# zailaiyiwan123/NOVA_pointcloud

Hardware: AMD Instinct MI355X
Metric: generated points/sec/node, NOVA-d48w1024 @2048 pts, 64-step sample (higher is better)
Workload: dtype bf16; 1 GPU; d48w1024_2048pts_b32; ar_steps=64, diffusion_steps=25, batch_per_gpu=32, global_batch=32, guidance=cfg 2-pass, process_group=none

## Files before the change

### include/nova_hip.h

```cpp
#ifndef NOVA_HIP_H_
#define NOVA_HIP_H_

#ifdef __cplusplus
extern "C" {
#endif

#define NOVA_HIP_VERSION 403

typedef enum { NOVA_F32 = 0, NOVA_BF16 = 1, NOVA_F16 = 2 } nova_dtype;
typedef enum { NOVA_ACT_NONE = 0, NOVA_ACT_GELU_ERF = 1, NOVA_ACT_SILU = 2 } nova_act;
typedef enum {
  NOVA_OK = 0,
  NOVA_ERR_ARG = -1,
  NOVA_ERR_SHAPE = -2,
  NOVA_ERR_LAUNCH = -3,
  NOVA_ERR_DEVICE = -4
} nova_status;

int nova_version(void);
const char* nova_last_error(void);
int nova_check_device(void);

#define NOVA_PROF_SLOTS 10
int nova_prof_enable(int on);
int nova_prof_collect(double* ms, double* work, long long* launches, int slots);

int nova_debug_force_gemm_tile(int tile);

int nova_debug_set_attn_variant(int variant);

int nova_debug_set_graphs(int on);
int nova_debug_graph_stats(long* captures, long* replays);
int nova_debug_drop_graphs(void);

int nova_gemm_bias_act(const void* A, const void* W, const float* bias, void* out, int M, int N, int K, int act,
                       int dtype, void* stream);

int nova_quantize_rows_fp8(const void* x_bf16, void* out_fp8, float* scale, long long rows, int D, void* stream);
int nova_gemm_fp8_bias_act(const void* A8, const float* a_scale, const void* W8, const float* w_scale, const float* bias,
                           void* out_bf16, int M, int N, int K, int act, void* stream);

int nova_qkv_rope(const void* x, const void* Wqkv, const float* bias, const float* rope, void* qkv, int S, int L, int D,
                  int heads, int rope_batch, int dtype, void* stream);

int nova_qkv_rope_cols(const void* x, const void* W, const float* bias, const float* rope, void* out, int M, int N, int K,
                       int L, int rope_batch, int head_dim, int rope_cols, int dtype, void* stream);

int nova_rope_table(const float* pos, const long long* ids, float* rope, int nb, int pad, int n_tok, int n_pos, int hd,
                    const float* inv_freq, void* stream);

int nova_attn_fwd(const void* q, const void* k, const void* v, void* o, int S, int heads, int Lq, int Lk, int head_dim,
                  long q_row_stride, long kv_row_stride, long o_row_stride, float scale, int dtype, void* stream);

int nova_attn_fwd_lse(const void* q_scaled, const void* k, const void* v, void* o, float* lse, int S, int heads, int L,
                      int head_dim, long qkv_row_stride, long o_row_stride, const int* key_limit, void* stream);
int nova_attn_bwd(const void* q_scaled, const void* k, const void* v, const void* o, const void* d_o, const float* lse,
                  float* delta_scratch, void* dq, void* dk, void* dv, int S, int heads, int L, int head_dim,
                  long qkv_row_stride, long o_row_stride, long do_row_stride, long dqkv_row_stride, float scale,
                  const int* key_limit, void* stream);

int nova_act_fwd(const void* x, void* y, long long n, int kind, int dtype, void* stream);
int nova_act_bwd(const void* x, const void* dy, void* dx, long long n, int kind, int dtype, void* stream);

int nova_row_norm_bwd(const void* x, const void* dy, const float* gamma, const float* beta, const void* mod, long mod_ld,
                      int scale_off, int shift_off, int gate_off, void* dx, void* dmod, float* dgamma_part, float* dbeta_part,
                      int parts, long rows, int D, float eps, int dtype, void* stream);

int nova_row_norm(const void* in, void* out, const float* gamma, const float* beta, const void* mod, long mod_ld,
                  int scale_off, int shift_off, int gate_off, const void* res, const int* gather, long rows, int D,
                  float eps, int dtype, void* stream);

int nova_row_norm_chain(const void* g, const void* x, const float* gamma, const float* beta, const void* mod, long mod_ld,
                        int gate_off, int scale_off, int shift_off, float eps_first, float eps_second, void* x_new_out,
                        void* h_out, long rows, int D, int dtype, void* stream);

int nova_adaln_fc1(const void* x, const void* mod, long mod_ld, int scale_off, int shift_off, float eps, const void* w,
                   const float* bias, void* h, void* out, long rows, int N, int D, int act, int dtype, void* stream);

int nova_embed_canvas(const float* canvas, const float* mask, const void* w, const float* bias, const void* mask_token,
                      const void* pos_embed, void* z0, int B, int N, int P, int D, int dtype, void* stream);
// ... 105 lines not shown
```

### nova_pointcloud_amd/csrc/capi.hip

```cpp
#include <cstdarg>
#include <cstdio>
#include <cstring>
#include <atomic>
#include <cmath>
#include <cstdlib>
#include <mutex>
#include <string>
#include <unordered_map>
#include <utility>
#include <vector>
#include "common.h"
#include "nova_internal.h"

namespace nova {

static thread_local char g_err[512] = "";

int set_error(int code, const char* fmt, ...) {
  va_list ap;
  va_start(ap, fmt);
  vsnprintf(g_err, sizeof(g_err), fmt, ap);
  va_end(ap);
  return code;
}

int check_launch(const char* what) {
  const hipError_t e = hipGetLastError();
  if (e == hipSuccess) return 0;
  return set_error(NOVA_ERR_LAUNCH, "%s: %s", what, hipGetErrorString(e));
}

struct ProfRec { hipEvent_t a, b; int slot; double work; };
static std::atomic<bool> g_prof_on{false};
static std::mutex g_prof_mu;
static std::vector<ProfRec> g_prof;
static std::vector<std::pair<hipEvent_t, hipEvent_t>> g_prof_pool;

ProfScope::ProfScope(int slot, double work, hipStream_t s) : idx(-1), st(s) {
  if (!g_prof_on.load(std::memory_order_relaxed)) return;
  std::lock_guard<std::mutex> lk(g_prof_mu);
  ProfRec r;
  if (!g_prof_pool.empty()) {
    r.a = g_prof_pool.back().first;
    r.b = g_prof_pool.back().second;
    g_prof_pool.pop_back();
  } else if (hipEventCreate(&r.a) != hipSuccess || hipEventCreate(&r.b) != hipSuccess) {
    return;
  }
  r.slot = slot;
  r.work = work;
  (void)hipEventRecord(r.a, st);
  g_prof.push_back(r);
  idx = (int)g_prof.size() - 1;
}
ProfScope::~ProfScope() {
  if (idx < 0) return;
  std::lock_guard<std::mutex> lk(g_prof_mu);
  if (idx < (int)g_prof.size()) (void)hipEventRecord(g_prof[idx].b, st);
}

static inline bool bad_dtype(int dtype) { return dtype != NOVA_F32 && dtype != NOVA_BF16 && dtype != NOVA_F16; }
static inline size_t esize(int dtype) { return dtype_is16(dtype) ? 2 : 4; }

}

using namespace nova;

#define NOVA_REQUIRE(cond, code, ...) \
  do {                                \
    if (!(cond)) return set_error(code, __VA_ARGS__); \
  } while (0)
#define NOVA_TRY(expr)        \
  do {                        \
    const int rc_ = (expr);   \
    if (rc_ != 0) return rc_; \
  } while (0)

namespace nova {
static thread_local bool g_walk_rev = false;
void walk_reverse(bool on) { g_walk_rev = on; }
bool walk_is_reverse() { return g_walk_rev; }
#ifdef NOVA_EXPERIMENTS
static int g_walk_alternate = 1;
void walk_set_alternate(int on) { g_walk_alternate = on; }
#else
constexpr int g_walk_alternate = 1;
#endif
}

extern "C" {

int nova_version(void) { return NOVA_HIP_VERSION; }
const char* nova_last_error(void) { return g_err; }

int nova_check_device(void) {
  int dev = -1;
  if (hipGetDevice(&dev) != hipSuccess) return set_error(NOVA_ERR_DEVICE, "no HIP device");
  hipDeviceProp_t prop;
  if (hipGetDeviceProperties(&prop, dev) != hipSuccess) return set_error(NOVA_ERR_DEVICE, "hipGetDeviceProperties failed");
  if (strncmp(prop.gcnArchName, "gfx950", 6) != 0)
    return set_error(NOVA_ERR_DEVICE, "device %d is %s; libnova_hip is built for gfx950 only", dev, prop.gcnArchName);
  return 0;
}

int nova_debug_force_gemm_tile(int tile) {
  NOVA_REQUIRE(gemm_force_tile(tile) == 0, NOVA_ERR_ARG,
               "force_gemm_tile: this build knows 0 (auto), 16 (small-M kernel; 161 / 162 / 164 with 16 / 32 / 64 rows per workgroup), 64 / 128 (the small-M tile kernels), 256 (persistent), 257 (one tile per workgroup) and 258 (persistent, prologue form); experiment codes need the NOVA_EXPERIMENTS build");
  return 0;
}

int nova_prof_enable(int on) {
  g_prof_on.store(on != 0);
  return 0;
}

int nova_prof_collect(double* ms, double* work, long long* launches, int slots) {
  NOVA_REQUIRE(ms && work && launches && slots >= PROF_SLOTS, NOVA_ERR_ARG, "prof_collect: need %d slots", PROF_SLOTS);
  for (int i = 0; i < slots; ++i) { ms[i] = 0; work[i] = 0; launches[i] = 0; }
  std::lock_guard<std::mutex> lk(g_prof_mu);
  for (auto& r : g_prof) {
    float t = 0.f;
    if (hipEventSynchronize(r.b) == hipSuccess && hipEventElapsedTime(&t, r.a, r.b) == hipSuccess) {
      ms[r.slot] += t;
      work[r.slot] += r.work;
      launches[r.slot] += 1;
    }
    g_prof_pool.emplace_back(r.a, r.b);
  }
  g_prof.clear();
  return 0;
}

int nova_gemm_bias_act(const void* A, const void* W, const float* bias, void* out, int M, int N, int K, int act,
                       int dtype, void* stream) {
  NOVA_REQUIRE(!bad_dtype(dtype), NOVA_ERR_ARG, "gemm: bad dtype %d", dtype);
  NOVA_REQUIRE(M == 0 || (A && W && out), NOVA_ERR_ARG, "gemm: null pointer");
  return gemm_bias_act(A, W, bias, out, M, N, K, act, dtype, (hipStream_t)stream);
}

int nova_quantize_rows_fp8(const void* x, void* out, float* scale, long long rows, int D, void* stream) {
  NOVA_REQUIRE(rows <= 0 || (x && out && scale), NOVA_ERR_ARG, "quantize_rows_fp8: null pointer");
  return quantize_rows_fp8(x, out, scale, (long)rows, D, (hipStream_t)stream);
}

int nova_gemm_fp8_bias_act(const void* A8, const float* a_scale, const void* W8, const float* w_scale, const float* bias,
                           void* out, int M, int N, int K, int act, void* stream) {
  NOVA_REQUIRE(M <= 0 || (A8 && a_scale && W8 && w_scale && out), NOVA_ERR_ARG, "gemm_fp8: null pointer");
  NOVA_REQUIRE(act >= NOVA_ACT_NONE && act <= NOVA_ACT_SILU, NOVA_ERR_ARG, "gemm_fp8: bad activation %d", act);
  return gemm256_fp8_launch(A8, a_scale, W8, w_scale, bias, out, M, N, K, act, (hipStream_t)stream);
}

int nova_qkv_rope(const void* x, const void* Wqkv, const float* bias, const float* rope, void* qkv, int S, int L, int D,
                  int heads, int rope_batch, int dtype, void* stream) {
  NOVA_REQUIRE(!bad_dtype(dtype), NOVA_ERR_ARG, "qkv_rope: bad dtype %d", dtype);
  NOVA_REQUIRE(S * L == 0 || (x && Wqkv && qkv), NOVA_ERR_ARG, "qkv_rope: null pointer");
  return gemm_qkv_rope(x, Wqkv, bias, rope, qkv, S, L, D, heads, rope_batch, dtype, (hipStream_t)stream);
}

int nova_qkv_rope_cols(const void* x, const void* W, const float* bias, const float* rope, void* out, int M, int N, int K,
                       int L, int rope_batch, int head_dim, int rope_cols, int dtype, void* stream) {
// ... 530 lines not shown
```

### nova_pointcloud_amd/csrc/gemm.hip

```cpp
#include <cstdlib>
#include "common.h"
#include "nova_internal.h"

namespace nova {

constexpr int ROWB = 128;

struct GemmEpi {
  const float* bias;
  const float* rope;
  int L;
  int rope_batch;
  int hd;
  int rope_cols;
  float q_scale;
  int q_cols;
};

enum { EPI_NONE = 0, EPI_GELU = 1, EPI_SILU = 2, EPI_ROPE = 3 };

template <typename T> struct Frag;
template <> struct Frag<bf16_t> { u4v v; };
template <> struct Frag<f16_t> { u4v v; };
template <> struct Frag<float> { f4v v; };

__device__ __forceinline__ f4v mma(const Frag<bf16_t>& w, const Frag<bf16_t>& a, f4v c) { return Half16<bf16_t>::mfma16(w.v, a.v, c); }
__device__ __forceinline__ f4v mma(const Frag<f16_t>& w, const Frag<f16_t>& a, f4v c) { return Half16<f16_t>::mfma16(w.v, a.v, c); }
__device__ __forceinline__ f4v mma(const Frag<float>& w, const Frag<float>& a, f4v c) {
#pragma unroll
  for (int j = 0; j < 4; ++j) c = __builtin_amdgcn_mfma_f32_16x16x4f32(w.v[j], a.v[j], c, 0, 0, 0);
  return c;
}

template <typename T>
__device__ __forceinline__ Frag<T> lds_frag(const char* tile, int row, int chunk) {
  const int phys = chunk ^ ((row >> 1) & 7);
  Frag<T> f;
  f.v = *reinterpret_cast<const decltype(f.v)*>(tile + row * ROWB + phys * 16);
  return f;
}

#ifndef NOVA_GEMM64_STAGES
#define NOVA_GEMM64_STAGES 2
#endif
template <typename T, int EPI, int F = 4>
__global__ __launch_bounds__(256, 2) void gemm_kernel(const T* __restrict__ A, const T* __restrict__ W,
                                                       T* __restrict__ C, int M, int N, int K, int ntm,
                                                       int ntn, GemmEpi e) {
  constexpr int BM = 32 * F, BN = 32 * F, TILE_BYTES = BM * ROWB, WT = 16 * F;
  constexpr int NST = F == 2 ? NOVA_GEMM64_STAGES : 2;
  __shared__ __attribute__((aligned(16))) char smem[NST * 2 * TILE_BYTES];
  const int tid = threadIdx.x, lane = tid & 63, wid = tid >> 6;
  const int wm = wid >> 1, wn = wid & 1;

  const int nwg = ntm * ntn;
  const int t = xcd_remap(blockIdx.x, nwg);
  constexpr int GM = 8;
  const int per_group = GM * ntn;
  const int group = t / per_group, first_m = group * GM;
  const int gsz = min(ntm - first_m, GM);
  const int tm = first_m + (t % per_group) % gsz;
  const int tn = (t % per_group) / gsz;
  const int m0 = tm * BM, n0 = tn * BN;

  const int rr = lane >> 3, cp = lane & 7;
  const char* a_src[4];
  const char* w_src[4];
  const size_t rowbytes = (size_t)K * sizeof(T);
#pragma unroll
// ... 20 lines not shown
  f4v bv[F];
#pragma unroll
  for (int nf = 0; nf < F; ++nf) bv[nf] = f4v{0.f, 0.f, 0.f, 0.f};
  if (e.bias) {
#pragma unroll
    for (int nf = 0; nf < F; ++nf) bv[nf] = *reinterpret_cast<const f4v*>(e.bias + n0 + wn * WT + nf * 16 + fg * 4);
  }
  f4v acc[F][F];
#pragma unroll
  for (int i = 0; i < F; ++i)
#pragma unroll
    for (int j = 0; j < F; ++j) acc[i][j] = bv[i];

#pragma unroll
  for (int s = 0; s < NST - 1; ++s)
    if (s < nkt) stage(s, s);
  for (int kt = 0; kt < nkt; ++kt) {
    if constexpr (NST == 2) {
      asm volatile("s_waitcnt vmcnt(0)" ::: "memory");
    } else {
      const int young = min(NST - 2, nkt - 1 - kt);
      if (young >= 3) asm volatile("s_waitcnt vmcnt(%0)" ::"n"(3 * 2 * F) : "memory");
      else if (young == 2) asm volatile("s_waitcnt vmcnt(%0)" ::"n"(2 * 2 * F) : "memory");
      else if (young == 1) asm volatile("s_waitcnt vmcnt(%0)" ::"n"(1 * 2 * F) : "memory");
      else asm volatile("s_waitcnt vmcnt(0)" ::: "memory");
    }
    if constexpr (NST == 2) __syncthreads();
    else asm volatile("s_barrier" ::: "memory");
    if (kt + NST - 1 < nkt) stage((kt + NST - 1) % NST, kt + NST - 1);
    const char* ta = smem + (kt % NST) * 2 * TILE_BYTES;
    const char* tw = ta + TILE_BYTES;
#pragma unroll
    for (int kk = 0; kk < 2; ++kk) {
      Frag<T> af[F], wf[F];
#pragma unroll
      for (int f = 0; f < F; ++f) {
        af[f] = lds_frag<T>(ta, wm * WT + f * 16 + fr, fg + 4 * kk);
        wf[f] = lds_frag<T>(tw, wn * WT + f * 16 + fr, fg + 4 * kk);
      }
#pragma unroll
      for (int nf = 0; nf < F; ++nf)
#pragma unroll
        for (int mf = 0; mf < F; ++mf) acc[nf][mf] = mma(wf[nf], af[mf], acc[nf][mf]);
    }
  }

  const bool rot = EPI == EPI_ROPE && n0 < e.rope_cols;
#pragma unroll
  for (int mf = 0; mf < F; ++mf) {
    const int m = m0 + wm * WT + mf * 16 + fr;
    if (m >= M) continue;
    f4v cs[F];
    if (rot) {
      const int s = m / e.L, l = m - s * e.L;
      const float* ropem = e.rope + ((size_t)(s % e.rope_batch) * e.L + l) * e.hd;
#pragma unroll
      for (int nf = 0; nf < F; ++nf) cs[nf] = *reinterpret_cast<const f4v*>(ropem + (n0 + wn * WT + nf * 16 + fg * 4) % e.hd);
    }
    T* dst = C + (size_t)m * N + n0 + wn * WT + fg * 4;
#pragma unroll
    for (int nf = 0; nf < F; ++nf) {
      f4v v = acc[nf][mf];
      if (EPI == EPI_GELU) {
#pragma unroll
        for (int j = 0; j < 4; ++j) v[j] = sizeof(T) == 2 ? v[j] : gelu_erf(v[j]);
        if (sizeof(T) == 2) v = gelu_erf_fast4(v);
      } else if (EPI == EPI_SILU) {
#pragma unroll
        for (int j = 0; j < 4; ++j) v[j] = silu(v[j]);
      } else if (EPI == EPI_ROPE) {
        if (rot) {
          v = rope_rotate4(v, cs[nf]);
        }
        if (n0 < e.q_cols) v = v * e.q_scale;
      }
      if constexpr (sizeof(T) == 2) {
        u2v o = {Half16<T>::pack(v[0], v[1]), Half16<T>::pack(v[2], v[3])};
        *reinterpret_cast<u2v*>(dst + nf * 16) = o;
      } else {
        *reinterpret_cast<f4v*>(dst + nf * 16) = v;
      }
    }
  }
}

int gemm256_launch(const void* A, const void* W, void* C, int M, int N, int K, int epi, const float* bias,
                   const float* rope, int L, int rope_batch, int hd, int rope_cols, float q_scale, int q_cols, int dtype,
                   hipStream_t st, int form = 0);
int gemm256_cu_count();

static thread_local int g_force_tile = 0;
#ifdef NOVA_EXPERIMENTS
void gemm256_set_variant(int v);
void gemm256_set_gm(int g);
void gemm256_set_stagger(int cycles);
void gemm256_set_grid(int n);
void walk_set_alternate(int on);
#endif
int gemm_forced_tile() { return g_force_tile; }
int gemm_force_tile(int tile) {
#ifdef NOVA_EXPERIMENTS
  if (tile == 50000 || tile == 50001) {
    walk_set_alternate(tile - 50000);
    return 0;
  }
  if (tile >= 40000 && tile <= 40512) {
    gemm256_set_grid(tile - 40000);
    return 0;
  }
  if (tile >= 30000 && tile < 31000) {
    gemm256_set_stagger((tile - 30000) * 256);
    return 0;
  }
  if (tile >= 7001 && tile <= 7064) {
    gemm256_set_gm(tile - 7000);
    return 0;
  }
  if (tile >= 2560 && tile <= 2580) {
    gemm256_set_variant(tile - 2560);
    tile = 256;
  }
#endif
  if (tile == 161 || tile == 162 || tile == 164) {
    skinny_force_row_blocks(tile - 160);
    tile = 16;
  } else {
    skinny_force_row_blocks(0);
  }
  if (tile != 0 && tile != 16 && tile != 64 && tile != 128 && tile != 256 && tile != 257 && tile != 258) return -1;
  g_force_tile = tile;
  return 0;
}

static long min_tiles256() {
  static const long v = [] {
    const char* e = getenv("NOVA_GEMM_MIN_TILES");
    return e && *e ? atol(e) : (long)gemm256_cu_count() / 2;
  }();
  return v;
}

template <typename T>
static int launch_gemm(const void* A, const void* W, void* C, int M, int N, int K, int epi, const GemmEpi& e,
                       hipStream_t st) {
  const int kelems = ROWB / (int)sizeof(T);
  if (M <= 0) return 0;
  if (N % 128 != 0 || K % kelems != 0 || K <= 0)
    return set_error(NOVA_ERR_SHAPE, "gemm: need N %% 128 == 0 and K %% %d == 0 (got M=%d N=%d K=%d)", kelems, M, N, K);
  const bool can256 = N % 256 == 0 && (epi != EPI_ROPE || (e.rope_cols % 256 == 0 && e.q_cols % 256 == 0));
  if (g_force_tile >= 256 && !can256) return set_error(NOVA_ERR_SHAPE, "gemm: 256-tile kernel needs N %% 256 == 0");
  const long tiles256 = (long)((M + 255) / 256) * (N / 256);
  if (can256 && (g_force_tile >= 256 || (g_force_tile == 0 && M >= 4096 && tiles256 >= min_tiles256())))
    return gemm256_launch(A, W, C, M, N, K, epi, e.bias, e.rope, e.L, e.rope_batch, e.hd, e.rope_cols, e.q_scale, e.q_cols,
                          dtype_of<T>(), st, g_force_tile == 257 ? 1 : g_force_tile == 258 ? 2 : 0);
  constexpr int BM = 128, BN = 128;
  int ntm = (M + BM - 1) / BM, ntn = N / BN;
  ProfScope prof(PROF_GEMM_SMALL, 2.0 * M * N * K, st);
  const T* a = static_cast<const T*>(A);
  const T* w = static_cast<const T*>(W);
  T* c = static_cast<T*>(C);
  static const bool tile64_ok = [] { const char* v = getenv("NOVA_GEMM_TILE64"); return !(v && v[0] == '0'); }();
  if (g_force_tile == 64 || (tile64_ok && g_force_tile == 0 && epi != EPI_ROPE && (long)ntm * ntn * 4 <= (long)gemm256_cu_count() * 3)) {
    if (epi == EPI_ROPE) return set_error(NOVA_ERR_SHAPE, "gemm: the 64 tile has no RoPE epilogue");
    ntm = (M + 63) / 64;
    ntn = N / 64;
    dim3 grid64(ntm * ntn), block(256);
    switch (epi) {
      case EPI_NONE: hipLaunchKernelGGL((gemm_kernel<T, EPI_NONE, 2>), grid64, block, 0, st, a, w, c, M, N, K, ntm, ntn, e); break;
      case EPI_GELU: hipLaunchKernelGGL((gemm_kernel<T, EPI_GELU, 2>), grid64, block, 0, st, a, w, c, M, N, K, ntm, ntn, e); break;
      case EPI_SILU: hipLaunchKernelGGL((gemm_kernel<T, EPI_SILU, 2>), grid64, block, 0, st, a, w, c, M, N, K, ntm, ntn, e); break;
      default: return set_error(NOVA_ERR_ARG, "gemm: unknown epilogue %d", epi);
    }
    return check_launch("gemm (64 tile)");
  }
  dim3 grid(ntm * ntn), block(256);
  switch (epi) {
    case EPI_NONE: hipLaunchKernelGGL((gemm_kernel<T, EPI_NONE>), grid, block, 0, st, a, w, c, M, N, K, ntm, ntn, e); break;
    case EPI_GELU: hipLaunchKernelGGL((gemm_kernel<T, EPI_GELU>), grid, block, 0, st, a, w, c, M, N, K, ntm, ntn, e); break;
    case EPI_SILU: hipLaunchKernelGGL((gemm_kernel<T, EPI_SILU>), grid, block, 0, st, a, w, c, M, N, K, ntm, ntn, e); break;
    case EPI_ROPE: hipLaunchKernelGGL((gemm_kernel<T, EPI_ROPE>), grid, block, 0, st, a, w, c, M, N, K, ntm, ntn, e); break;
    default: return set_error(NOVA_ERR_ARG, "gemm: unknown epilogue %d", epi);
  }
  return check_launch("gemm");
}

int gemm_bias_act(const void* A, const void* W, const float* bias, void* out, int M, int N, int K, int act,
                  int dtype, hipStream_t st) {
  GemmEpi e{bias, nullptr, 1, 1, 2, 0, 1.0f, 0};
  if (act < 0 || act > 2) return set_error(NOVA_ERR_ARG, "gemm: unknown activation %d", act);
  if (dtype_is16(dtype) && (g_force_tile == 16 || (g_force_tile == 0 && skinny_gemm_fits(M, N, K, false))))
    return skinny_gemm(A, W, bias, out, M, N, K, act, nullptr, dtype, st);
  return dispatch_dtype(dtype, [&](auto tag) { return launch_gemm<decltype(tag)>(A, W, out, M, N, K, act, e, st); });
}

bool gemm_modulate_fused(int M, int N, int K, int dtype) {
  return dtype_is16(dtype) && (g_force_tile == 16 || (g_force_tile == 0 && skinny_gemm_fits(M, N, K, true)));
}

int gemm_modulate_act(const RowNormArgs& pro, const void* W, const float* bias, void* out, int M, int N, int K, int act,
                      int dtype, hipStream_t st) {
  if (gemm_modulate_fused(M, N, K, dtype)) return skinny_gemm(nullptr, W, bias, out, M, N, K, act, &pro, dtype, st);
  if (int rc = row_norm(pro, dtype, st)) return rc;
  return gemm_bias_act(pro.out, W, bias, out, M, N, K, act, dtype, st);
}

int gemm_qkv_rope(const void* x, const void* Wqkv, const float* bias, const float* rope, void* qkv, int S, int L,
                  int D, int heads, int rope_batch, int dtype, hipStream_t st, float q_scale) {
  const int hd = D / heads;
  if (heads <= 0 || D % heads != 0 || hd % 4 != 0) return set_error(NOVA_ERR_SHAPE, "qkv_rope: bad heads/D");
  const int epi = (rope || q_scale != 1.0f) ? EPI_ROPE : EPI_NONE;
  if (rope && rope_batch <= 0) return set_error(NOVA_ERR_ARG, "qkv_rope: rope_batch must be > 0");
  GemmEpi e{bias, rope, L, rope ? rope_batch : 1, hd, rope ? 2 * D : 0, q_scale, q_scale != 1.0f ? D : 0};
  return dispatch_dtype(dtype, [&](auto tag) { return launch_gemm<decltype(tag)>(x, Wqkv, qkv, S * L, 3 * D, D, epi, e, st); });
}

int gemm_rope_cols(const void* x, const void* W, const float* bias, const float* rope, void* out, int M, int N, int K,
                   int L, int rope_batch, int hd, int rope_cols, int dtype, hipStream_t st) {
  if (rope && rope_batch <= 0) return set_error(NOVA_ERR_ARG, "rope_cols: rope_batch must be > 0");
  GemmEpi e{bias, rope, L, rope ? rope_batch : 1, hd, rope_cols, 1.0f, 0};
  const int epi = rope ? EPI_ROPE : EPI_NONE;
  return dispatch_dtype(dtype, [&](auto tag) { return launch_gemm<decltype(tag)>(x, W, out, M, N, K, epi, e, st); });
}

}
```

### nova_pointcloud_amd/csrc/gemm256.hip

```cpp
#include <type_traits>
#ifndef NOVA_GEMM_ACT_ROWS
#define NOVA_GEMM_ACT_ROWS 1
#endif
#include "common.h"
#include "nova_internal.h"

namespace nova {

constexpr int P_UNIT = 128 * 128;
constexpr int P_BUF = 4 * P_UNIT;
constexpr int P_KLDS = 2 * P_BUF;
constexpr int P_BIAS = P_KLDS;
constexpr int P_LDS = P_KLDS + 1024;

struct GemmEpi;
struct GemmEpi256 {
  const float* bias;
  const float* rope;
  int L, rope_batch, hd, rope_cols;
  float q_scale;
  int q_cols;
  int gm;
  int rev;
  const float* sa;
// ... 932 lines not shown
#ifdef NOVA_EXPERIMENTS
static int g_gm256 = 8;
static int g_stagger256 = 0;
void gemm256_set_stagger(int cycles) { g_stagger256 = cycles; }
void gemm256_set_gm(int g) { g_gm256 = g; }
static int g_var256 = 20;
void gemm256_set_variant(int v) { g_var256 = v; }
#else
constexpr int g_gm256 = 8;
constexpr int g_stagger256 = 0;
constexpr int g_var256 = 20;
#endif

template <typename T, int VAR>
static int launch256v(const void* A, const void* W, void* C, int M, int N, int K, int epi, const GemmEpi256& e,
                     hipStream_t st) {
  const int ntm = (M + 255) / 256, ntn = N / 256;
  dim3 grid(ntm * ntn), block(512);
  ProfScope prof(prof_gemm_slot(epi, N, K), 2.0 * M * N * K, st);
  const T* a = static_cast<const T*>(A);
  const T* w = static_cast<const T*>(W);
  T* c = static_cast<T*>(C);
  switch (epi) {
    case E_NONE: hipLaunchKernelGGL((gemm256_kernel<T, E_NONE, VAR>), grid, block, 0, st, a, w, c, M, N, K, ntm, ntn, e); break;
    case E_GELU: hipLaunchKernelGGL((gemm256_kernel<T, E_GELU, VAR>), grid, block, 0, st, a, w, c, M, N, K, ntm, ntn, e); break;
    case E_SILU: hipLaunchKernelGGL((gemm256_kernel<T, E_SILU, VAR>), grid, block, 0, st, a, w, c, M, N, K, ntm, ntn, e); break;
    case E_ROPE: hipLaunchKernelGGL((gemm256_kernel<T, E_ROPE, VAR>), grid, block, 0, st, a, w, c, M, N, K, ntm, ntn, e); break;
    default: return set_error(NOVA_ERR_ARG, "gemm256: unknown epilogue %d", epi);
  }
  return check_launch("gemm256");
}

#ifdef NOVA_EXPERIMENTS
static int g_grid256 = 0;
void gemm256_set_grid(int n) { g_grid256 = n & ~7; }
#else
constexpr int g_grid256 = 0;
#endif
static int cu_slots() {
  if (g_grid256 > 0) return g_grid256;
  static int n = 0;
  if (n == 0) {
    int dev = 0, cus = 0;
    if (hipGetDevice(&dev) != hipSuccess || hipDeviceGetAttribute(&cus, hipDeviceAttributeMultiprocessorCount, dev) != hipSuccess || cus < 8) cus = 256;
    n = cus & ~7;
  }
  return n;
}

int gemm256_cu_count() { return cu_slots(); }

template <typename T>
static int launch256p(const void* A, const void* W, void* C, int M, int N, int K, int epi, const GemmEpi256& e,
                      hipStream_t st) {
  const int ntm = (M + 255) / 256, ntn = N / 256;
  dim3 grid(cu_slots()), block(512);
  ProfScope prof(prof_gemm_slot(epi, N, K), 2.0 * M * N * K, st);
  const T* a = static_cast<const T*>(A);
  const T* w = static_cast<const T*>(W);
  T* c = static_cast<T*>(C);
  switch (epi) {
    case E_NONE: hipLaunchKernelGGL((gemm256p_kernel<T, E_NONE>), grid, block, 0, st, a, w, c, M, N, K, ntm, ntn, e); break;
    case E_GELU: hipLaunchKernelGGL((gemm256p_kernel<T, E_GELU>), grid, block, 0, st, a, w, c, M, N, K, ntm, ntn, e); break;
    case E_SILU: hipLaunchKernelGGL((gemm256p_kernel<T, E_SILU>), grid, block, 0, st, a, w, c, M, N, K, ntm, ntn, e); break;
    case E_ROPE: hipLaunchKernelGGL((gemm256p_kernel<T, E_ROPE>), grid, block, 0, st, a, w, c, M, N, K, ntm, ntn, e); break;
    default: return set_error(NOVA_ERR_ARG, "gemm256: unknown epilogue %d", epi);
  }
  return check_launch("gemm256p");
}

int gemm256_fp8_launch(const void* A8, const float* sa, const void* W8, const float* sw, const float* bias, void* C, int M,
                       int N, int K, int epi, hipStream_t st, const float* rope, int L, int rope_batch, int hd, int rope_cols,
                       float q_scale, int q_cols, int sa_scalar, const float* q8_scale, unsigned* q8_amax) {
  if (M <= 0) return 0;
  if (N % 256 != 0 || K % 128 != 0 || K <= 0) return set_error(NOVA_ERR_SHAPE, "gemm_fp8: need N %% 256 == 0 and K %% 128 == 0 (got N=%d K=%d)", N, K);
  if (epi == E_ROPE && (rope_cols % 256 || q_cols % 256 || (rope && (L < 16 || rope_batch <= 0 || hd <= 0))))
    return set_error(NOVA_ERR_SHAPE, "gemm_fp8: RoPE epilogue needs rope_cols, q_cols %% 256 == 0 and L >= 16");
  GemmEpi256 e{bias, rope, rope ? L : 1, rope ? rope_batch : 1, rope ? hd : 2, rope ? rope_cols : 0, q_scale, q_cols, g_gm256,
               walk_is_reverse() ? 1 : 0, sa, sw, 0};
  e.sa_scalar = sa_scalar;
  e.q8_scale = q8_scale;
  e.q8_amax = q8_amax;
  if (epi == E_GELU_Q8 && (!q8_scale || !q8_amax)) return set_error(NOVA_ERR_ARG, "gemm_fp8: the e4m3-output epilogue needs a scale and an amax word");
  const int ntm = (M + 255) / 256, ntn = N / 256;
  dim3 grid(cu_slots()), block(512);
  ProfScope prof(prof_gemm_slot(epi == E_GELU_Q8 ? E_GELU : epi, N, K), 2.0 * M * N * K, st);
  const fp8_t* a = static_cast<const fp8_t*>(A8);
  const fp8_t* w = static_cast<const fp8_t*>(W8);
  bf16_t* c = static_cast<bf16_t*>(C);
  switch (epi) {
    case E_NONE: hipLaunchKernelGGL((gemm256p_kernel<fp8_t, E_NONE>), grid, block, 0, st, a, w, c, M, N, K, ntm, ntn, e); break;
    case E_GELU: hipLaunchKernelGGL((gemm256p_kernel<fp8_t, E_GELU>), grid, block, 0, st, a, w, c, M, N, K, ntm, ntn, e); break;
    case E_SILU: hipLaunchKernelGGL((gemm256p_kernel<fp8_t, E_SILU>), grid, block, 0, st, a, w, c, M, N, K, ntm, ntn, e); break;
    case E_ROPE: hipLaunchKernelGGL((gemm256p_kernel<fp8_t, E_ROPE>), grid, block, 0, st, a, w, c, M, N, K, ntm, ntn, e); break;
    case E_GELU_Q8: hipLaunchKernelGGL((gemm256p_kernel<fp8_t, E_GELU_Q8>), grid, block, 0, st, a, w, c, M, N, K, ntm, ntn, e); break;
    default: return set_error(NOVA_ERR_ARG, "gemm_fp8: unknown epilogue %d", epi);
  }
  return check_launch("gemm256p fp8");
}

template <typename T>
static int launch256c(const void* A, const void* W, void* C, int M, int N, int K, int epi, const GemmEpi256& e,
                      hipStream_t st) {
  const int ntm = (M + 255) / 256, ntn = N / 256;
  dim3 grid(cu_slots()), block(512);
  ProfScope prof(prof_gemm_slot(epi, N, K), 2.0 * M * N * K, st);
  const T* a = static_cast<const T*>(A);
  const T* w = static_cast<const T*>(W);
  T* c = static_cast<T*>(C);
  switch (epi) {
    case E_NONE: hipLaunchKernelGGL((gemm256c_kernel<T, E_NONE>), grid, block, 0, st, a, w, c, M, N, K, ntm, ntn, e); break;
    case E_GELU: hipLaunchKernelGGL((gemm256c_kernel<T, E_GELU>), grid, block, 0, st, a, w, c, M, N, K, ntm, ntn, e); break;
    case E_SILU: hipLaunchKernelGGL((gemm256c_kernel<T, E_SILU>), grid, block, 0, st, a, w, c, M, N, K, ntm, ntn, e); break;
    case E_ROPE:
      if (e.rope && e.hd == 64) hipLaunchKernelGGL((gemm256c_kernel<T, E_ROPE, true>), grid, block, 0, st, a, w, c, M, N, K, ntm, ntn, e);
      else hipLaunchKernelGGL((gemm256c_kernel<T, E_ROPE, false>), grid, block, 0, st, a, w, c, M, N, K, ntm, ntn, e);
      break;
    default: return set_error(NOVA_ERR_ARG, "gemm256: unknown epilogue %d", epi);
  }
  return check_launch("gemm256c");
}

template <typename T>
static int launch256(const void* A, const void* W, void* C, int M, int N, int K, int epi, const GemmEpi256& e,
                     hipStream_t st, int form) {
  if (form != 1 && g_var256 == 20 && !(epi == E_ROPE && e.rope && e.L < 16)) {
    const int nkt = K / (128 / (int)sizeof(T));
    if (form == 0 && nkt >= 4 && (nkt & 1) == 0) return launch256c<T>(A, W, C, M, N, K, epi, e, st);
    return launch256p<T>(A, W, C, M, N, K, epi, e, st);
  }
#ifdef NOVA_EXPERIMENTS
  switch (g_var256) {
    case 1: return launch256v<T, 1>(A, W, C, M, N, K, epi, e, st);
    case 3: return launch256v<T, 3>(A, W, C, M, N, K, epi, e, st);
    case 0: return launch256v<T, 0>(A, W, C, M, N, K, epi, e, st);
    case 10: return launch256v<T, 10>(A, W, C, M, N, K, epi, e, st);
    case 11: return launch256v<T, 11>(A, W, C, M, N, K, epi, e, st);
    case 12: return launch256v<T, 12>(A, W, C, M, N, K, epi, e, st);
    default: break;
  }
#endif
  return launch256v<T, 2>(A, W, C, M, N, K, epi, e, st);
}

int gemm256_launch(const void* A, const void* W, void* C, int M, int N, int K, int epi, const float* bias,
                   const float* rope, int L, int rope_batch, int hd, int rope_cols, float q_scale, int q_cols, int dtype,
                   hipStream_t st, int form) {
#ifdef NOVA_EXPERIMENTS
  const int gm = g_gm256;
#else
  const int gm = (N <= 1024 && K * (int)(dtype_is16(dtype) ? 2 : 4) <= 2048) ? 16 : g_gm256;
#endif
  GemmEpi256 e{bias, rope, L, rope_batch, hd, rope_cols, q_scale, q_cols, gm, walk_is_reverse() ? 1 : 0, nullptr, nullptr, g_stagger256};
  return dispatch_dtype(dtype, [&](auto tag) { return launch256<decltype(tag)>(A, W, C, M, N, K, epi, e, st, form); });
}

}
```

### nova_pointcloud_amd/csrc/nova_internal.h

```cpp
#pragma once
#include <hip/hip_runtime.h>
#include "../../include/nova_hip.h"

#include "common.h"

namespace nova {

template <typename T> constexpr int dtype_of() { return sizeof(T) == 4 ? NOVA_F32 : NOVA_BF16; }
template <> constexpr int dtype_of<f16_t>() { return NOVA_F16; }
inline bool dtype_is16(int dtype) { return dtype == NOVA_BF16 || dtype == NOVA_F16; }
template <typename F> inline auto dispatch_dtype(int dtype, F&& f) {
  return dtype == NOVA_BF16 ? f(bf16_t{}) : dtype == NOVA_F16 ? f(f16_t{}) : f(float{});
}
template <typename F> inline auto dispatch_half(int dtype, F&& f) { return dtype == NOVA_F16 ? f(f16_t{}) : f(bf16_t{}); }

int set_error(int code, const char* fmt, ...) __attribute__((format(printf, 2, 3)));
int check_launch(const char* what);

enum { PROF_GEMM_NONE = 0, PROF_GEMM_GELU, PROF_GEMM_SILU, PROF_GEMM_ROPE, PROF_ATTN, PROF_ROWNORM, PROF_GEMM_SMALL, PROF_GEMM_WIDEK,
       PROF_TOKENS, PROF_DECODER, PROF_SLOTS };
inline int prof_gemm_slot(int epi, int N, int K) { return epi == 0 && K > N ? PROF_GEMM_WIDEK : PROF_GEMM_NONE + epi; }
struct ProfScope {
  ProfScope(int slot, double work, hipStream_t st);
  ~ProfScope();
  int idx;
  hipStream_t st;
};

int gemm_bias_act(const void* A, const void* W, const float* bias, void* out, int M, int N, int K, int act,
                  int dtype, hipStream_t st);
int gemm_qkv_rope(const void* x, const void* Wqkv, const float* bias, const float* rope, void* qkv, int S, int L,
                  int D, int heads, int rope_batch, int dtype, hipStream_t st, float q_scale = 1.0f);

int gemm_rope_cols(const void* x, const void* W, const float* bias, const float* rope, void* out, int M, int N, int K,
                   int L, int rope_batch, int hd, int rope_cols, int dtype, hipStream_t st);
int gemm_force_tile(int tile);
int gemm_forced_tile();
void walk_reverse(bool on);
bool walk_is_reverse();

int attn_fwd(const void* q, const void* k, const void* v, void* o, int S, int heads, int Lq, int Lk, int hd,
             long q_row_stride, long kv_row_stride, long o_row_stride, float scale, int dtype, hipStream_t st,
             bool q_prescaled = false, long kv_seq_stride = 0, float* lse = nullptr, const int* klim = nullptr);
int attn_fwd_m16(const void* q, const void* k, const void* v, void* o, int S, int heads, int Lq, int Lk, int hd, long q_rs, long kv_rs,
                 long o_rs, float cl, int dtype, hipStream_t st, long kv_ss, float* lse, int rows_per_wave, bool sum_on_mfma, bool pipelined = false,
                 const int* klim = nullptr);
constexpr int NOVA_ATTN_DEFAULT_VARIANT = 3;
int attn_set_variant(int v);
int attn_variant();
int attn_bwd(const void* q, const void* k, const void* v, const void* o, const void* d_o, const float* lse, float* delta, void* dq,
             void* dk, void* dv, int S, int heads, int L, int hd, long qkv_rs, long o_rs, long do_rs, long dqkv_rs, float scale,
             hipStream_t st, const int* klim = nullptr);

struct RowNormArgs {
  const void* in;
  void* out;
  const float* gamma;
  const float* beta;
  const void* mod;
  long mod_ld;
  int scale_off, shift_off, gate_off;
  const void* res;
  const int* gather;
  long rows;
  int D;
  float eps;
  int rev = 0;
  void* out8 = nullptr;
  float* out8_scale = nullptr;
};
int row_norm(const RowNormArgs& a, int dtype, hipStream_t st);

bool skinny_gemm_fits(int M, int N, int K, bool modulate);
bool gemm_modulate_fused(int M, int N, int K, int dtype);
int skinny_forced_row_blocks();
void skinny_force_row_blocks(int rb);
int skinny_gemm(const void* A, const void* W, const float* bias, void* out, int M, int N, int K, int act,
                const RowNormArgs* pro, int dtype, hipStream_t st);
int row_norm_chain(const RowNormArgs& a2, const RowNormArgs& a1, void* x_new_out, int dtype, hipStream_t st);
int gemm_modulate_act(const RowNormArgs& pro, const void* W, const float* bias, void* out, int M, int N, int K, int act,
                      int dtype, hipStream_t st);

int rope_table(const float* pos, const long long* ids, float* table, int nb, int pad, int n_tok, int n_pos,
               int hd, const float* inv_freq, hipStream_t st);
int embed_canvas(const float* canvas, const float* mask, const void* w, const float* bias, const void* mask_token,
                 const void* pos_embed, void* z0, int B, int N, int P, int D, int dtype, hipStream_t st);
int build_sequence(const void* prefix, long prefix_seq_rows, const void* tokens, long tok_batch_rows,
                   const long long* ids, void* x, int S, int B, int Lp, int n_sel, int D, int dtype, hipStream_t st);
// ... 37 lines not shown
```

### nova_pointcloud_amd/hip.py

```python

import ctypes
import os
import threading

import torch

F32, BF16, F16 = 0, 1, 2
ACT_NONE, ACT_GELU_ERF, ACT_SILU = 0, 1, 2

_LIB_PATH = os.path.join(os.path.dirname(os.path.abspath(__file__)), "libnova_hip.so")
_lock = threading.Lock()
_lib = None
_device_ok = False

c_void_p, c_int, c_long, c_float = ctypes.c_void_p, ctypes.c_int, ctypes.c_long, ctypes.c_float


class NovaHipError(RuntimeError):
    """Raised when libnova_hip.so is missing, mis-built, or a call into it fails."""


class VitBlock(ctypes.Structure):

    _fields_ = [(k, c_void_p) for k in (
# ... 17 lines not shown
        "adaln_w", "adaln_b", "patch_w", "patch_b", "head_w", "head_b")]


class SamplerStep(ctypes.Structure):

    _fields_ = [(k, c_float) for k in ("guidance", "kx", "kv", "clip", "c0", "cx", "sigma", "extra_scale")] + [("extra_kind", c_int)]


SIGNATURES = {
    "nova_gemm_bias_act": [c_void_p] * 4 + [c_int] * 5 + [c_void_p],
    "nova_qkv_rope": [c_void_p] * 5 + [c_int] * 6 + [c_void_p],
    "nova_quantize_rows_fp8": [c_void_p] * 3 + [ctypes.c_longlong, c_int, c_void_p],
    "nova_gemm_fp8_bias_act": [c_void_p] * 6 + [c_int] * 4 + [c_void_p],
    "nova_qkv_rope_cols": [c_void_p] * 5 + [c_int] * 8 + [c_void_p],
    "nova_rope_table": [c_void_p] * 3 + [c_int] * 5 + [c_void_p, c_void_p],
    "nova_attn_fwd": [c_void_p] * 4 + [c_int] * 5 + [c_long] * 3 + [c_float, c_int, c_void_p],
    "nova_row_norm": [c_void_p] * 5 + [c_long] + [c_int] * 3 + [c_void_p, c_void_p, c_long, c_int, c_float, c_int, c_void_p],
    "nova_embed_canvas": [c_void_p] * 7 + [c_int] * 5 + [c_void_p],
    "nova_build_sequence": [c_void_p, c_long, c_void_p, c_long, c_void_p, c_void_p] + [c_int] * 6 + [c_void_p],
    "nova_scatter_tokens": [c_void_p] * 3 + [c_int] * 7 + [c_void_p],
    "nova_silu_add_rows": [c_void_p] * 3 + [c_long, c_int, c_int, c_void_p],
    "nova_timestep_freq": [c_void_p] * 3 + [c_int] * 3 + [c_void_p],
    "nova_patch_embed_rows": [c_void_p] * 4 + [c_int] * 6 + [c_void_p],
    "nova_head_cfg_euler": [c_void_p] * 4 + [c_int] * 4 + [c_float, c_int, c_float, c_int, c_void_p],
    "nova_vit_blocks_forward": [ctypes.POINTER(VitBlock), c_int, c_void_p] + [c_int] * 5 + [c_void_p, c_int]
    + [c_void_p] * 4 + [c_int, c_void_p],
    "nova_row_norm_fp8": [c_void_p] * 7 + [c_long, c_int, c_float, c_void_p],
    "nova_gemm_fp8_gelu_q8": [c_void_p] * 6 + [c_int] * 3 + [c_void_p, c_void_p, c_void_p],
    "nova_qkv_rope_fp8": [c_void_p] * 7 + [c_int] * 5 + [c_float, c_void_p],
    "nova_vit_blocks_forward_fp8": [ctypes.POINTER(VitBlock), ctypes.POINTER(VitBlockFp8), c_int, c_void_p] + [c_int] * 5
    + [c_void_p, c_int] + [c_void_p] * 10 + [c_void_p],
    "nova_vit_blocks_forward_kv": [ctypes.POINTER(VitBlock), c_int, c_void_p] + [c_int] * 5 + [c_void_p, c_int]
    + [c_void_p, c_long, c_long] + [c_void_p] * 4 + [c_int, c_void_p],
    "nova_pointset_nn_dist": [c_void_p] * 3 + [c_int] * 3 + [c_float, c_float, c_int, c_void_p],
    "nova_pointset_pairwise_dist": [c_void_p] * 3 + [c_int] * 3 + [c_float, c_float, c_void_p],
    "nova_pointset_chamfer_matrix": [c_void_p] * 3 + [c_int] * 6 + [c_void_p],
    "nova_pointset_emd_matrix": [c_void_p] * 3 + [c_int] * 4 + [c_void_p],
    "nova_modulate_rows": [c_void_p] * 3 + [c_long, c_int, c_int, c_void_p],
    "nova_attn_fwd_lse": [c_void_p] * 5 + [c_int, c_int, c_int, c_int, c_long, c_long, c_void_p, c_void_p],
    "nova_attn_bwd": [c_void_p] * 10 + [c_int, c_int, c_int, c_int, c_long, c_long, c_long, c_long, c_float, c_void_p, c_void_p],
    "nova_row_norm_bwd": [c_void_p] * 5 + [c_long, c_int, c_int, c_int] + [c_void_p] * 4 + [c_int, c_long, c_int, c_float, c_int, c_void_p],
    "nova_act_fwd": [c_void_p, c_void_p, ctypes.c_longlong, c_int, c_int, c_void_p],
    "nova_act_bwd": [c_void_p, c_void_p, c_void_p, ctypes.c_longlong, c_int, c_int, c_void_p],
    "nova_row_norm_chain": [c_void_p] * 5 + [c_long, c_int, c_int, c_int, c_float, c_float, c_void_p, c_void_p, c_long, c_int, c_int, c_void_p],
    "nova_adaln_fc1": [c_void_p, c_void_p, c_long, c_int, c_int, c_float, c_void_p, c_void_p, c_void_p, c_void_p, c_long]
    + [c_int] * 4 + [c_void_p],
    "nova_decoder_denoise": [ctypes.POINTER(Decoder), c_void_p, c_void_p, c_void_p, c_void_p, c_void_p, c_float, c_void_p]
    + [c_int] * 6 + [c_void_p] * 7 + [c_int, c_int, c_void_p],
    "nova_decoder_denoise_echo": [ctypes.POINTER(Decoder), c_void_p, c_void_p, c_void_p, c_void_p, c_void_p, c_float, c_void_p, c_void_p]
    + [c_int] * 7 + [c_void_p] * 7 + [c_int, c_int, c_void_p],
}
SIGNATURES["nova_prof_enable"] = [c_int]
SIGNATURES["nova_debug_force_gemm_tile"] = [c_int]
SIGNATURES["nova_debug_set_graphs"] = [c_int]
SIGNATURES["nova_debug_set_attn_variant"] = [c_int]
SIGNATURES["nova_debug_drop_graphs"] = []
SIGNATURES["nova_debug_graph_stats"] = [ctypes.POINTER(c_long), ctypes.POINTER(c_long)]
SIGNATURES["nova_prof_collect"] = [ctypes.POINTER(ctypes.c_double), ctypes.POINTER(ctypes.c_double),
                                   ctypes.POINTER(ctypes.c_longlong), c_int]
PROF_SLOTS = ["gemm_bias", "gemm_bias_gelu", "gemm_bias_silu", "qkv_gemm_rope", "attention", "row_norm", "gemm_small_tile", "gemm_bias_wide_k",
              "token_plumbing", "decoder_glue"]
PLAIN = {"nova_version": (c_int, []), "nova_last_error": (ctypes.c_char_p, []), "nova_check_device": (c_int, [])}


def lib_path() -> str:
    return _LIB_PATH


ABI_VERSION = 403


def load(check_device=True):
    global _lib, _device_ok
    with _lock:
        if _lib is None:
            if not os.path.exists(_LIB_PATH):
                raise NovaHipError(
                    f"{_LIB_PATH} not found: the HIP extension is not built. Run "
                    "`python -c 'import __graft_entry__ as g; g.build()'` (or `make -C nova_pointcloud_amd/csrc`). "
                    "There is no CPU fallback for the generation path."
                )
            try:
                lib = ctypes.CDLL(_LIB_PATH)
            except OSError as e:
                raise NovaHipError(f"cannot load {_LIB_PATH}: {e}") from e
            lib.nova_version.restype = c_int
            if lib.nova_version() != ABI_VERSION:
                raise NovaHipError(f"{_LIB_PATH} is C ABI version {lib.nova_version()}, this package binds version {ABI_VERSION} "
                                   "(include/nova_hip.h NOVA_HIP_VERSION): rebuild it with `make -C nova_pointcloud_amd/csrc`")
            for name, argtypes in SIGNATURES.items():
                fn = getattr(lib, name)
                fn.argtypes, fn.restype = argtypes, c_int
            for name, (res, argtypes) in PLAIN.items():
                fn = getattr(lib, name)
                fn.argtypes, fn.restype = argtypes, res
            _lib = lib
        if check_device and not _device_ok:
            if not torch.cuda.is_available():
                raise NovaHipError("no GPU visible: libnova_hip needs an MI355X (gfx950) device")
            rc = _lib.nova_check_device()
            if rc != 0:
                raise NovaHipError(_lib.nova_last_error().decode())
            _device_ok = True
    return _lib


def call(name, *args):
    lib = _lib if (_lib is not None and _device_ok) else load()
    rc = getattr(lib, name)(*args)
    if rc != 0:
        raise NovaHipError(f"{name} failed ({rc}): {lib.nova_last_error().decode()}")


def dtype_code(dtype: torch.dtype) -> int:
    if dtype == torch.float32:
        return F32
    if dtype == torch.bfloat16:
        return BF16
    if dtype == torch.float16:
        return F16
    raise NovaHipError(f"libnova_hip supports float32, bfloat16 and float16 activations, got {dtype}")

# ... 120 lines not shown
```

Before: 8184 points/s.

## Split partial last round of persistent 256-tile GEMM into smaller-tile tail launch

When the persistent 256-tile GEMM would end with a partially filled final round, a cost model now decides whether to cut the row panels there. The full rounds run on the 256 kernel, and the leftover rows go to a 128 or 64 tile kernel. A row offset is threaded into the epilogue so the RoPE indexing stays correct. This is meant to cut wave-quantization idle time on the last round, at the cost of an extra kernel launch and a heuristic timing model that may misjudge some shapes.

Result: no change. 8263 points/s, median of 6 (+1.0%).

```diff
diff --git a/include/nova_hip.h b/include/nova_hip.h
--- a/include/nova_hip.h
+++ b/include/nova_hip.h
@@ -5,7 +5,7 @@
 extern "C" {
 #endif
 
-#define NOVA_HIP_VERSION 403
+#define NOVA_HIP_VERSION 404
 
 typedef enum { NOVA_F32 = 0, NOVA_BF16 = 1, NOVA_F16 = 2 } nova_dtype;
 typedef enum { NOVA_ACT_NONE = 0, NOVA_ACT_GELU_ERF = 1, NOVA_ACT_SILU = 2 } nova_act;
@@ -26,6 +26,8 @@
 int nova_prof_collect(double* ms, double* work, long long* launches, int slots);
 
 int nova_debug_force_gemm_tile(int tile);
+
+int nova_debug_gemm_tail_plan(int M, int N, int K, int dtype, int epilogue, int cus, int force, int* plan);
 
 int nova_debug_set_attn_variant(int variant);
 
diff --git a/nova_pointcloud_amd/csrc/capi.hip b/nova_pointcloud_amd/csrc/capi.hip
--- a/nova_pointcloud_amd/csrc/capi.hip
+++ b/nova_pointcloud_amd/csrc/capi.hip
@@ -37,7 +37,7 @@
 static std::vector<std::pair<hipEvent_t, hipEvent_t>> g_prof_pool;
 
 ProfScope::ProfScope(int slot, double work, hipStream_t s) : idx(-1), st(s) {
-  if (!g_prof_on.load(std::memory_order_relaxed)) return;
+  if (slot < 0 || !g_prof_on.load(std::memory_order_relaxed)) return;
   std::lock_guard<std::mutex> lk(g_prof_mu);
   ProfRec r;
   if (!g_prof_pool.empty()) {
@@ -105,7 +105,17 @@
 
 int nova_debug_force_gemm_tile(int tile) {
   NOVA_REQUIRE(gemm_force_tile(tile) == 0, NOVA_ERR_ARG,
-               "force_gemm_tile: this build knows 0 (auto), 16 (small-M kernel; 161 / 162 / 164 with 16 / 32 / 64 rows per workgroup), 64 / 128 (the small-M tile kernels), 256 (persistent), 257 (one tile per workgroup) and 258 (persistent, prologue form); experiment codes need the NOVA_EXPERIMENTS build");
+               "force_gemm_tile: this build knows 0 (auto), 16 (small-M kernel; 161 / 162 / 164 with 16 / 32 / 64 rows per workgroup), 64 / 128 (the small-M tile kernels), 256 (persistent), 257 (one tile per workgroup) and 258 (persistent, prologue form), 300 .. 303 (row split of a partial last round of the persistent kernel: off / by rule / always / always on the 128 tile); experiment codes need the NOVA_EXPERIMENTS build");
+  return 0;
+}
+
+int nova_debug_gemm_tail_plan(int M, int N, int K, int dtype, int epilogue, int cus, int force, int* plan) {
+  NOVA_REQUIRE(plan && !bad_dtype(dtype), NOVA_ERR_ARG, "gemm_tail_plan: null pointer or bad dtype %d", dtype);
+  const GemmTailPlan p = gemm_tail_plan(M, N, K, (int)esize(dtype), epilogue, cus, force);
+  plan[0] = p.panels256;
+  plan[1] = p.tail_rows;
+  plan[2] = p.tail_tile;
+  plan[3] = (int)gemm256_rounds((long)((M + 255) / 256) * (N / 256), cus);
   return 0;
 }
 
diff --git a/nova_pointcloud_amd/csrc/gemm.hip b/nova_pointcloud_amd/csrc/gemm.hip
--- a/nova_pointcloud_amd/csrc/gemm.hip
+++ b/nova_pointcloud_amd/csrc/gemm.hip
@@ -15,6 +15,7 @@
   int rope_cols;
   float q_scale;
   int q_cols;
+  int row0 = 0;
 };
 
 enum { EPI_NONE = 0, EPI_GELU = 1, EPI_SILU = 2, EPI_ROPE = 3 };
@@ -141,7 +142,7 @@
     if (m >= M) continue;
     f4v cs[F];
     if (rot) {
-      const int s = m / e.L, l = m - s * e.L;
+      const int mg = e.row0 + m, s = mg / e.L, l = mg - s * e.L;
       const float* ropem = e.rope + ((size_t)(s % e.rope_batch) * e.L + l) * e.hd;
 #pragma unroll
       for (int nf = 0; nf < F; ++nf) cs[nf] = *reinterpret_cast<const f4v*>(ropem + (n0 + wn * WT + nf * 16 + fg * 4) % e.hd);
@@ -175,10 +176,11 @@
 
 int gemm256_launch(const void* A, const void* W, void* C, int M, int N, int K, int epi, const float* bias,
                    const float* rope, int L, int rope_batch, int hd, int rope_cols, float q_scale, int q_cols, int dtype,
-                   hipStream_t st, int form = 0);
+                   hipStream_t st, int form = 0, bool book = true);
 int gemm256_cu_count();
 
 static thread_local int g_force_tile = 0;
+static thread_local int g_tail_split = 1;
 #ifdef NOVA_EXPERIMENTS
 void gemm256_set_variant(int v);
 void gemm256_set_gm(int g);
@@ -186,8 +188,12 @@
 void gemm256_set_grid(int n);
 void walk_set_alternate(int on);
 #endif
-int gemm_forced_tile() { return g_force_tile; }
+int gemm_forced_tile() { return g_force_tile + ((g_tail_split ^ 1) << 20); }
 int gemm_force_tile(int tile) {
+  if (tile >= 300 && tile <= 303) {
+    g_tail_split = tile - 300;
+    return 0;
+  }
 #ifdef NOVA_EXPERIMENTS
   if (tile == 50000 || tile == 50001) {
     walk_set_alternate(tile - 50000);
@@ -227,6 +233,54 @@
     return e && *e ? atol(e) : (long)gemm256_cu_count() / 2;
   }();
   return v;
+}
+
+static double tail_kernel_us(int tile, long wgs, double kf) {
+  return tile == 64 ? 4.0 + 4.0 * kf + 0.0115 * kf * (double)wgs : 4.5 + 9.0 * kf + 0.022 * kf * (double)wgs;
+}
+long gemm256_rounds(long tiles, int cus) {
+  const long nslot = cus / 8;
+  return ((tiles + 7) / 8 + nslot - 1) / nslot;
+}
+GemmTailPlan gemm_tail_plan(int M, int N, int K, int elem_bytes, int epi, int cus, int force) {
+  GemmTailPlan plan{(M + 255) / 256, 0, 0};
+  if (M <= 0 || N <= 0 || N % 256 != 0 || K <= 0 || cus < 8) return plan;
+  const long ntm = plan.panels256, ntn = N / 256;
+  const long rounds = gemm256_rounds(ntm * ntn, cus);
+  if (rounds < 2 || ntm * ntn >= (long)(cus / 8) * 8 * rounds) return plan;
+  const long keep = (long)(cus / 8) * 8 * (rounds - 1) / ntn;
+  if (keep <= 0 || keep >= ntm) return plan;
+  const long rows = (long)M - keep * 256;
+  const double kf = (double)K * elem_bytes / 2048.0;
+  const double t128 = tail_kernel_us(128, ((rows + 127) / 128) * (N / 128), kf);
+  const double t64 = (epi == EPI_ROPE || force == 2) ? 1e30 : tail_kernel_us(64, ((rows + 63) / 64) * (N / 64), kf);
+  const double tail = t64 < t128 ? t64 : t128;
+  if (force == 0 && tail + 4.0 > 0.75 * (3.0 + 25.0 * kf)) return plan;
+  plan.panels256 = (int)keep;
+  plan.tail_rows = (int)rows;
+  plan.tail_tile = t64 < t128 ? 64 : 128;
+  return plan;
+}
+
+template <typename T, int F>
+static int launch_tile(const T* a, const T* w, T* c, int M, int N, int K, int epi, const GemmEpi& e, hipStream_t st) {
+  constexpr int BM = 32 * F;
+  const int ntm = (M + BM - 1) / BM, ntn = N / BM;
+  dim3 grid(ntm * ntn), block(256);
+  switch (epi) {
+    case EPI_NONE: hipLaunchKernelGGL((gemm_kernel<T, EPI_NONE, F>), grid, block, 0, st, a, w, c, M, N, K, ntm, ntn, e); break;
+    case EPI_GELU: hipLaunchKernelGGL((gemm_kernel<T, EPI_GELU, F>), grid, block, 0, st, a, w, c, M, N, K, ntm, ntn, e); break;
+    case EPI_SILU: hipLaunchKernelGGL((gemm_kernel<T, EPI_SILU, F>), grid, block, 0, st, a, w, c, M, N, K, ntm, ntn, e); break;
+    case EPI_ROPE:
+      if constexpr (F == 4) {
+        hipLaunchKernelGGL((gemm_kernel<T, EPI_ROPE, F>), grid, block, 0, st, a, w, c, M, N, K, ntm, ntn, e);
+        break;
+      } else {
+        return set_error(NOVA_ERR_SHAPE, "gemm: the 64 tile has no RoPE epilogue");
+      }
+    default: return set_error(NOVA_ERR_ARG, "gemm: unknown epilogue %d", epi);
+  }
+  return check_launch(F == 2 ? "gemm (64 tile)" : "gemm");
 }
 
 template <typename T>
@@ -238,39 +292,33 @@
     return set_error(NOVA_ERR_SHAPE, "gemm: need N %% 128 == 0 and K %% %d == 0 (got M=%d N=%d K=%d)", kelems, M, N, K);
   const bool can256 = N % 256 == 0 && (epi != EPI_ROPE || (e.rope_cols % 256 == 0 && e.q_cols % 256 == 0));
   if (g_force_tile >= 256 && !can256) return set_error(NOVA_ERR_SHAPE, "gemm: 256-tile kernel needs N %% 256 == 0");
-  const long tiles256 = (long)((M + 255) / 256) * (N / 256);
-  if (can256 && (g_force_tile >= 256 || (g_force_tile == 0 && M >= 4096 && tiles256 >= min_tiles256())))
-    return gemm256_launch(A, W, C, M, N, K, epi, e.bias, e.rope, e.L, e.rope_batch, e.hd, e.rope_cols, e.q_scale, e.q_cols,
-                          dtype_of<T>(), st, g_force_tile == 257 ? 1 : g_force_tile == 258 ? 2 : 0);
-  constexpr int BM = 128, BN = 128;
-  int ntm = (M + BM - 1) / BM, ntn = N / BN;
-  ProfScope prof(PROF_GEMM_SMALL, 2.0 * M * N * K, st);
   const T* a = static_cast<const T*>(A);
   const T* w = static_cast<const T*>(W);
   T* c = static_cast<T*>(C);
+  const long tiles256 = (long)((M + 255) / 256) * (N / 256);
+  if (can256 && (g_force_tile >= 256 || (g_force_tile == 0 && M >= 4096 && tiles256 >= min_tiles256()))) {
+    const int form = g_force_tile == 257 ? 1 : g_force_tile == 258 ? 2 : 0;
+    GemmTailPlan plan{0, 0, 0};
+    if (g_tail_split && form != 1) plan = gemm_tail_plan(M, N, K, (int)sizeof(T), epi, gemm256_cu_count(), g_tail_split - 1);
+    if (plan.tail_rows <= 0)
+      return gemm256_launch(A, W, C, M, N, K, epi, e.bias, e.rope, e.L, e.rope_batch, e.hd, e.rope_cols, e.q_scale, e.q_cols,
+                            dtype_of<T>(), st, form);
+    ProfScope prof(prof_gemm_slot(epi, N, K), 2.0 * M * N * K, st);
+    const int m1 = plan.panels256 * 256;
+    if (int rc = gemm256_launch(A, W, C, m1, N, K, epi, e.bias, e.rope, e.L, e.rope_batch, e.hd, e.rope_cols, e.q_scale, e.q_cols,
+                                dtype_of<T>(), st, form, false))
+      return rc;
+    GemmEpi et = e;
+    et.row0 = e.row0 + m1;
+    if (plan.tail_tile == 64) return launch_tile<T, 2>(a + (size_t)m1 * K, w, c + (size_t)m1 * N, plan.tail_rows, N, K, epi, et, st);
+    return launch_tile<T, 4>(a + (size_t)m1 * K, w, c + (size_t)m1 * N, plan.tail_rows, N, K, epi, et, st);
+  }
+  ProfScope prof(PROF_GEMM_SMALL, 2.0 * M * N * K, st);
   static const bool tile64_ok = [] { const char* v = getenv("NOVA_GEMM_TILE64"); return !(v && v[0] == '0'); }();
-  if (g_force_tile == 64 || (tile64_ok && g_force_tile == 0 && epi != EPI_ROPE && (long)ntm * ntn * 4 <= (long)gemm256_cu_count() * 3)) {
-    if (epi == EPI_ROPE) return set_error(NOVA_ERR_SHAPE, "gemm: the 64 tile has no RoPE epilogue");
-    ntm = (M + 63) / 64;
-    ntn = N / 64;
-    dim3 grid64(ntm * ntn), block(256);
-    switch (epi) {
-      case EPI_NONE: hipLaunchKernelGGL((gemm_kernel<T, EPI_NONE, 2>), grid64, block, 0, st, a, w, c, M, N, K, ntm, ntn, e); break;
-      case EPI_GELU: hipLaunchKernelGGL((gemm_kernel<T, EPI_GELU, 2>), grid64, block, 0, st, a, w, c, M, N, K, ntm, ntn, e); break;
-      case EPI_SILU: hipLaunchKernelGGL((gemm_kernel<T, EPI_SILU, 2>), grid64, block, 0, st, a, w, c, M, N, K, ntm, ntn, e); break;
-      default: return set_error(NOVA_ERR_ARG, "gemm: unknown epilogue %d", epi);
-    }
-    return check_launch("gemm (64 tile)");
-  }
-  dim3 grid(ntm * ntn), block(256);
-  switch (epi) {
-    case EPI_NONE: hipLaunchKernelGGL((gemm_kernel<T, EPI_NONE>), grid, block, 0, st, a, w, c, M, N, K, ntm, ntn, e); break;
-    case EPI_GELU: hipLaunchKernelGGL((gemm_kernel<T, EPI_GELU>), grid, block, 0, st, a, w, c, M, N, K, ntm, ntn, e); break;
-    case EPI_SILU: hipLaunchKernelGGL((gemm_kernel<T, EPI_SILU>), grid, block, 0, st, a, w, c, M, N, K, ntm, ntn, e); break;
-    case EPI_ROPE: hipLaunchKernelGGL((gemm_kernel<T, EPI_ROPE>), grid, block, 0, st, a, w, c, M, N, K, ntm, ntn, e); break;
-    default: return set_error(NOVA_ERR_ARG, "gemm: unknown epilogue %d", epi);
-  }
-  return check_launch("gemm");
+  const long tiles128 = (long)((M + 127) / 128) * (N / 128);
+  if (g_force_tile == 64 || (tile64_ok && g_force_tile == 0 && epi != EPI_ROPE && tiles128 * 4 <= (long)gemm256_cu_count() * 3))
+    return launch_tile<T, 2>(a, w, c, M, N, K, epi, e, st);
+  return launch_tile<T, 4>(a, w, c, M, N, K, epi, e, st);
 }
 
 int gemm_bias_act(const void* A, const void* W, const float* bias, void* out, int M, int N, int K, int act,
diff --git a/nova_pointcloud_amd/csrc/gemm256.hip b/nova_pointcloud_amd/csrc/gemm256.hip
--- a/nova_pointcloud_amd/csrc/gemm256.hip
+++ b/nova_pointcloud_amd/csrc/gemm256.hip
@@ -1008,10 +1008,10 @@
 
 template <typename T>
 static int launch256p(const void* A, const void* W, void* C, int M, int N, int K, int epi, const GemmEpi256& e,
-                      hipStream_t st) {
+                      hipStream_t st, bool book) {
   const int ntm = (M + 255) / 256, ntn = N / 256;
   dim3 grid(cu_slots()), block(512);
-  ProfScope prof(prof_gemm_slot(epi, N, K), 2.0 * M * N * K, st);
+  ProfScope prof(book ? prof_gemm_slot(epi, N, K) : -1, 2.0 * M * N * K, st);
   const T* a = static_cast<const T*>(A);
   const T* w = static_cast<const T*>(W);
   T* c = static_cast<T*>(C);
@@ -1057,10 +1057,10 @@
 
 template <typename T>
 static int launch256c(const void* A, const void* W, void* C, int M, int N, int K, int epi, const GemmEpi256& e,
-                      hipStream_t st) {
+                      hipStream_t st, bool book) {
   const int ntm = (M + 255) / 256, ntn = N / 256;
   dim3 grid(cu_slots()), block(512);
-  ProfScope prof(prof_gemm_slot(epi, N, K), 2.0 * M * N * K, st);
+  ProfScope prof(book ? prof_gemm_slot(epi, N, K) : -1, 2.0 * M * N * K, st);
   const T* a = static_cast<const T*>(A);
   const T* w = static_cast<const T*>(W);
   T* c = static_cast<T*>(C);
@@ -1079,11 +1079,11 @@
 
 template <typename T>
 static int launch256(const void* A, const void* W, void* C, int M, int N, int K, int epi, const GemmEpi256& e,
-                     hipStream_t st, int form) {
+                     hipStream_t st, int form, bool book) {
   if (form != 1 && g_var256 == 20 && !(epi == E_ROPE && e.rope && e.L < 16)) {
     const int nkt = K / (128 / (int)sizeof(T));
-    if (form == 0 && nkt >= 4 && (nkt & 1) == 0) return launch256c<T>(A, W, C, M, N, K, epi, e, st);
-    return launch256p<T>(A, W, C, M, N, K, epi, e, st);
+    if (form == 0 && nkt >= 4 && (nkt & 1) == 0) return launch256c<T>(A, W, C, M, N, K, epi, e, st, book);
+    return launch256p<T>(A, W, C, M, N, K, epi, e, st, book);
   }
 #ifdef NOVA_EXPERIMENTS
   switch (g_var256) {
@@ -1101,14 +1101,14 @@
 
 int gemm256_launch(const void* A, const void* W, void* C, int M, int N, int K, int epi, const float* bias,
                    const float* rope, int L, int rope_batch, int hd, int rope_cols, float q_scale, int q_cols, int dtype,
-                   hipStream_t st, int form) {
+                   hipStream_t st, int form, bool book) {
 #ifdef NOVA_EXPERIMENTS
   const int gm = g_gm256;
 #else
   const int gm = (N <= 1024 && K * (int)(dtype_is16(dtype) ? 2 : 4) <= 2048) ? 16 : g_gm256;
 #endif
   GemmEpi256 e{bias, rope, L, rope_batch, hd, rope_cols, q_scale, q_cols, gm, walk_is_reverse() ? 1 : 0, nullptr, nullptr, g_stagger256};
-  return dispatch_dtype(dtype, [&](auto tag) { return launch256<decltype(tag)>(A, W, C, M, N, K, epi, e, st, form); });
-}
-
-}
+  return dispatch_dtype(dtype, [&](auto tag) { return launch256<decltype(tag)>(A, W, C, M, N, K, epi, e, st, form, book); });
+}
+
+}
diff --git a/nova_pointcloud_amd/csrc/nova_internal.h b/nova_pointcloud_amd/csrc/nova_internal.h
--- a/nova_pointcloud_amd/csrc/nova_internal.h
+++ b/nova_pointcloud_amd/csrc/nova_internal.h
@@ -34,6 +34,9 @@
 
 int gemm_rope_cols(const void* x, const void* W, const float* bias, const float* rope, void* out, int M, int N, int K,
                    int L, int rope_batch, int hd, int rope_cols, int dtype, hipStream_t st);
+struct GemmTailPlan { int panels256, tail_rows, tail_tile; };
+GemmTailPlan gemm_tail_plan(int M, int N, int K, int elem_bytes, int epi, int cus, int force = 0);
+long gemm256_rounds(long tiles, int cus);
 int gemm_force_tile(int tile);
 int gemm_forced_tile();
 void walk_reverse(bool on);
diff --git a/nova_pointcloud_amd/hip.py b/nova_pointcloud_amd/hip.py
--- a/nova_pointcloud_amd/hip.py
+++ b/nova_pointcloud_amd/hip.py
@@ -93,6 +93,7 @@
 }
 SIGNATURES["nova_prof_enable"] = [c_int]
 SIGNATURES["nova_debug_force_gemm_tile"] = [c_int]
+SIGNATURES["nova_debug_gemm_tail_plan"] = [c_int] * 7 + [ctypes.POINTER(c_int)]
 SIGNATURES["nova_debug_set_graphs"] = [c_int]
 SIGNATURES["nova_debug_set_attn_variant"] = [c_int]
 SIGNATURES["nova_debug_drop_graphs"] = []
@@ -108,7 +109,7 @@
     return _LIB_PATH
 
 
-ABI_VERSION = 403
+ABI_VERSION = 404
 
 
 def load(check_device=True):
```
